# astaka-pe/Dual-DMP

Measured on NVIDIA B200. Metric: train iters/s (dual GCN fwd+bwd+loss+clip+Adam), higher is better.
Workload: dtype f32

## Files before the change

dual_dmp_b200/csrc/gemm_tc.cu:

```cuda
#include <cuda.h>
#include <cuda_fp16.h>
#include <stdlib.h>

#include <atomic>
#include <type_traits>

#include "common.cuh"

namespace ddmp {
namespace tc {

constexpr int kProducerWarps = 8;
constexpr int kProducerThreads = kProducerWarps * 32;
constexpr int BM = 128;
constexpr int BK = 32;
constexpr int UMMA_K = 8;

__device__ __forceinline__ uint32_t smem_u32(const void* p) { return (uint32_t)__cvta_generic_to_shared(p); }

__device__ __forceinline__ void mbar_init(uint64_t* bar, uint32_t count) {
    asm volatile("mbarrier.init.shared::cta.b64 [%0], %1;" ::"r"(smem_u32(bar)), "r"(count));
}
__device__ __forceinline__ void mbar_arrive(uint64_t* bar) {
    asm volatile("mbarrier.arrive.shared::cta.b64 _, [%0];" ::"r"(smem_u32(bar)) : "memory");
// ... 583 lines not shown
    auto load = [&](float4 (&buf)[NJ], uint32_t& vmask, int& k0) {
        k0 = lc_kb * BK16;
        vmask = 0;
#pragma unroll
        for (int j = 0; j < NJ; ++j) {
            if (rp[j]) {
                buf[j] = ldg4_pinned(rp[j] + k0);
                vmask |= 1u << j;
            } else {
                buf[j] = make_float4(0.f, 0.f, 0.f, 0.f);
            }
        }
        if (++lc_kb == num_kb) {
            lc_kb = 0;
            lc_tile += tile_step;
            if (lc_tile < g.num_tiles) set_rows(lc_tile);
        }
    };
    auto process = [&](float4 (&buf)[NJ], uint32_t vmask, int k0, uint32_t it) {
        const int s = it % STAGES;
        const uint32_t ph = (it / STAGES) & 1;
        const bool tr = g.trace && blockIdx.x == 0 && t == 0;
        long long c1 = 0, c2 = 0, c3 = 0;
        float4 sc = make_float4(s_a, s_a, s_a, s_a), sh = make_float4(0.f, 0.f, 0.f, 0.f);
        if (has_act) {
            sc = ldg4(g.scale + k0 + c8);
            sh = ldg4(g.shift + k0 + c8);
            sc.x *= s_a; sc.y *= s_a; sc.z *= s_a; sc.w *= s_a;
            sh.x *= s_a; sh.y *= s_a; sh.z *= s_a; sh.w *= s_a;
        }
        if (tr) c1 = clock64();
        wait_empty(empty_bar + s, ph ^ 1u);
        if (tr) c2 = clock64();
        const uint32_t st = smem_base + s * stage_bytes;
#pragma unroll
        for (int j = 0; j < NJ; ++j) {
            const uint32_t row = (t >> 4) + j * RPP;
            float4 a = buf[j];
            if (has_act) {
                if (vmask & (1u << j)) {
                    a.x = lrelu_max(fmaf(a.x, sc.x, sh.x), g.slope); a.y = lrelu_max(fmaf(a.y, sc.y, sh.y), g.slope);
                    a.z = lrelu_max(fmaf(a.z, sc.z, sh.z), g.slope); a.w = lrelu_max(fmaf(a.w, sc.w, sh.w), g.slope);
                }
            } else {
                a.x *= s_a; a.y *= s_a; a.z *= s_a; a.w *= s_a;
            }
            uint32_t h0, l0, h1, l1;
            split_f16x2(a.x, a.y, h0, l0);
            split_f16x2(a.z, a.w, h1, l1);
            const uint32_t off = sw128(row, c4 >> 1) + ((c4 & 1u) << 3);
            sts64(st + off, h0, h1);
            sts64(st + a_bytes + off, l0, l1);
        }
        long long cA = 0, cB = 0;
        if (tr) cA = clock64();
        fence_proxy_async();
        if (tr) cB = clock64();
        __syncwarp();
        if (tr) c3 = clock64();
        if (lane == 0) mbar_arrive(full_bar + s);
        if (tr) {
            g.trace[1] += (unsigned long long)(c2 - c1);
            g.trace[2] += (unsigned long long)(c3 - c2);
            g.trace[3] += 1ull;
            g.trace[14] += (unsigned long long)(cA - c2);
            g.trace[15] += (unsigned long long)(cB - cA);
        }
    };
    float4 buf0[NJ], buf1[NJ];
    uint32_t vm0 = 0, vm1 = 0;
    int k0 = 0, k1 = 0;
    if (total > 0) {
        set_rows(lc_tile);
        load(buf0, vm0, k0);
    }
    for (uint32_t it = 0; it < total; it += 2) {
        if (it + 1 < total) load(buf1, vm1, k1);
        process(buf0, vm0, k0, it);
        if (it + 1 >= total) break;
        if (it + 2 < total) load(buf0, vm0, k0);
        process(buf1, vm1, k1, it + 1);
    }
}
__device__ __forceinline__ void tmem_ld32_async(uint32_t taddr, uint32_t (&v)[32]) {
    asm volatile(
        "tcgen05.ld.sync.aligned.32x32b.x32.b32 "
        "{%0, %1, %2, %3, %4, %5, %6, %7, %8, %9, %10, %11, %12, %13, %14, %15, "
        "%16, %17, %18, %19, %20, %21, %22, %23, %24, %25, %26, %27, %28, %29, %30, %31}, [%32];\n"
        : "=r"(v[0]), "=r"(v[1]), "=r"(v[2]), "=r"(v[3]), "=r"(v[4]), "=r"(v[5]), "=r"(v[6]), "=r"(v[7]), "=r"(v[8]),
          "=r"(v[9]), "=r"(v[10]), "=r"(v[11]), "=r"(v[12]), "=r"(v[13]), "=r"(v[14]), "=r"(v[15]), "=r"(v[16]),
          "=r"(v[17]), "=r"(v[18]), "=r"(v[19]), "=r"(v[20]), "=r"(v[21]), "=r"(v[22]), "=r"(v[23]), "=r"(v[24]),
          "=r"(v[25]), "=r"(v[26]), "=r"(v[27]), "=r"(v[28]), "=r"(v[29]), "=r"(v[30]), "=r"(v[31])
        : "r"(taddr)
        : "memory");
}
__device__ __forceinline__ void tmem_wait_ld() { asm volatile("tcgen05.wait::ld.sync.aligned;" ::: "memory"); }

template <class Args>
__device__ __forceinline__ void epilogue_block32(const Args& g, uint32_t (&v)[32], float inv_sa, uint32_t stg, int lane,
                                                 int64_t mrow0, int ncol0) {
    const int cc = lane & 7;
    float4 w = ldg4(g.inv_sw + ncol0 + cc * 4);
    if (g.flags & 8) {
        const int64_t m = mrow0 + lane;
        if (m < g.M) {
#pragma unroll
            for (int i = 0; i < 8; ++i) {
                const float4 ws = ldg4(g.inv_sw + ncol0 + 4 * i);
                st4(g.C + m * g.N + ncol0 + 4 * i,
                    make_float4(__uint_as_float(v[4 * i]) * inv_sa * ws.x, __uint_as_float(v[4 * i + 1]) * inv_sa * ws.y,
                                __uint_as_float(v[4 * i + 2]) * inv_sa * ws.z, __uint_as_float(v[4 * i + 3]) * inv_sa * ws.w));
            }
        }
        return;
    }
#pragma unroll
    for (int i = 0; i < 8; ++i)
        sts128(stg + (uint32_t)lane * 128u + (uint32_t)((i ^ (lane & 7)) << 4),
               make_uint4(v[4 * i], v[4 * i + 1], v[4 * i + 2], v[4 * i + 3]));
    w.x *= inv_sa; w.y *= inv_sa; w.z *= inv_sa; w.w *= inv_sa;
    __syncwarp();
    uint4 o[8];
#pragma unroll
    for (int j = 0; j < 8; ++j) {
        const int r = j * 4 + (lane >> 3);
        asm volatile("ld.shared.v4.b32 {%0, %1, %2, %3}, [%4];"
                     : "=r"(o[j].x), "=r"(o[j].y), "=r"(o[j].z), "=r"(o[j].w)
                     : "r"(stg + (uint32_t)r * 128u + (uint32_t)((cc ^ (r & 7)) << 4)));
    }
#pragma unroll
    for (int j = 0; j < 8; ++j) {
        const int64_t m = mrow0 + j * 4 + (lane >> 3);
        if (m < g.M)
            st4(g.C + m * g.N + ncol0 + cc * 4,
                make_float4(__uint_as_float(o[j].x) * w.x, __uint_as_float(o[j].y) * w.y,
                            __uint_as_float(o[j].z) * w.z, __uint_as_float(o[j].w) * w.w));
    }
    __syncwarp();
}
template <int BN, class Args>
__device__ __forceinline__ void epilogue_tile(const Args& g, uint32_t taddr, float inv_sa, uint32_t stg, int lane,
                                              int64_t mrow0, int n0) {
    static_assert(BN % 64 == 0, "two 32-column blocks per iteration");
    uint32_t va[32], vb[32];
    tmem_ld32_async(taddr, va);
#pragma unroll 1
    for (int cb = 0; cb < BN; cb += 64) {
        const bool tr = g.trace && blockIdx.x == 0 && threadIdx.x == 12 * 32;
        long long q0 = 0;
        if (tr) q0 = clock64();
        tmem_wait_ld();
        if (tr) g.trace[13] += (unsigned long long)(clock64() - q0);
        tmem_ld32_async(taddr + (uint32_t)cb + 32u, vb);
        epilogue_block32(g, va, inv_sa, stg, lane, mrow0, n0 + cb);
        tmem_wait_ld();
        if (cb + 64 < BN) tmem_ld32_async(taddr + (uint32_t)cb + 64u, va);
        epilogue_block32(g, vb, inv_sa, stg, lane, mrow0, n0 + cb + 32);
    }
}

__device__ __forceinline__ void tma_store_2d(const CUtensorMap* map, uint32_t src_smem, int c0, int c1) {
    asm volatile("cp.async.bulk.tensor.2d.global.shared::cta.tile.bulk_group [%0, {%1, %2}], [%3];" ::"l"(map), "r"(c0),
                 "r"(c1), "r"(src_smem)
                 : "memory");
}
__device__ __forceinline__ void bulk_commit() { asm volatile("cp.async.bulk.commit_group;" ::: "memory"); }
// ... 11 lines not shown
#pragma unroll
    for (int i = 0; i < 8; ++i)
        sts128(stg + (uint32_t)lane * 128u + (uint32_t)((i ^ (lane & 7)) << 4),
               make_uint4(__float_as_uint(__uint_as_float(v[4 * i]) * (cs[i].x * inv_sa)),
                          __float_as_uint(__uint_as_float(v[4 * i + 1]) * (cs[i].y * inv_sa)),
                          __float_as_uint(__uint_as_float(v[4 * i + 2]) * (cs[i].z * inv_sa)),
                          __float_as_uint(__uint_as_float(v[4 * i + 3]) * (cs[i].w * inv_sa))));
    fence_proxy_async();
    __syncwarp();
    if (lane == 0) {
        tma_store_2d(cmap, stg, ncol0, mrow0);
        bulk_commit();
    }
}
template <int BN>
__device__ __forceinline__ void epilogue_tile_tma(const CUtensorMap* cmap, const float* __restrict__ inv_sw, uint32_t taddr,
                                                  float inv_sa, uint32_t stg, int lane, int64_t mrow0, int n0) {
    static_assert(BN % 64 == 0, "two 32-column blocks per iteration");
    uint32_t va[32], vb[32];
    float4 cs[8];
    tmem_ld32_async(taddr, va);
#pragma unroll 1
    for (int cb = 0; cb < BN; cb += 64) {
#pragma unroll
        for (int i = 0; i < 8; ++i) cs[i] = ldg4(inv_sw + n0 + cb + 4 * i);
        tmem_wait_ld();
        tmem_ld32_async(taddr + (uint32_t)cb + 32u, vb);
        store_block32_tma(cmap, va, cs, inv_sa, stg, lane, (int)mrow0, n0 + cb);
#pragma unroll
        for (int i = 0; i < 8; ++i) cs[i] = ldg4(inv_sw + n0 + cb + 32 + 4 * i);
        tmem_wait_ld();
        if (cb + 64 < BN) tmem_ld32_async(taddr + (uint32_t)cb + 64u, va);
        store_block32_tma(cmap, vb, cs, inv_sa, stg + 32u * 128u, lane, (int)mrow0, n0 + cb + 32);
    }
}

__global__ void tc_prep_b16_kernel(const float* __restrict__ W, int transposed, uint8_t* __restrict__ img,
                                   float* __restrict__ inv_sw, int N, int K, int BN) {
    const int n = (int)(((int64_t)blockIdx.x * blockDim.x + threadIdx.x) >> 5);
    const int lane = threadIdx.x & 31;
    if (n >= N) return;
    const int chunks = K / 8;
    auto load8 = [&](int c, float4& a, float4& b) {
        const int k = c * 8;
        if (!transposed) {
            a = ldg4(W + (int64_t)n * K + k);
            b = ldg4(W + (int64_t)n * K + k + 4);
        } else {
            a.x = __ldg(W + (int64_t)(k + 0) * N + n); a.y = __ldg(W + (int64_t)(k + 1) * N + n);
            a.z = __ldg(W + (int64_t)(k + 2) * N + n); a.w = __ldg(W + (int64_t)(k + 3) * N + n);
            b.x = __ldg(W + (int64_t)(k + 4) * N + n); b.y = __ldg(W + (int64_t)(k + 5) * N + n);
            b.z = __ldg(W + (int64_t)(k + 6) * N + n); b.w = __ldg(W + (int64_t)(k + 7) * N + n);
        }
    };
    uint32_t m = 0;
    for (int c = lane; c < chunks; c += 32) {
        float4 a, b;
        load8(c, a, b);
        const float mx = fmaxf(fmaxf(fmaxf(fabsf(a.x), fabsf(a.y)), fmaxf(fabsf(a.z), fabsf(a.w))),
                               fmaxf(fmaxf(fabsf(b.x), fabsf(b.y)), fmaxf(fabsf(b.z), fabsf(b.w))));
        const uint32_t bits = __float_as_uint(mx);
        m = bits > m ? bits : m;
    }
    m = __reduce_max_sync(0xffffffffu, m);
    float s, inv_s;
    scale_from_bits(m, s, inv_s);
    if (lane == 0) inv_sw[n] = inv_s;
    const int n_tile = n / BN, r = n % BN, num_kb = K / BK16;
    const int64_t half_bytes = (int64_t)BN * 128;
    for (int c = lane; c < chunks; c += 32) {
        float4 a, b;
        load8(c, a, b);
        a.x *= s; a.y *= s; a.z *= s; a.w *= s; b.x *= s; b.y *= s; b.z *= s; b.w *= s;
        uint4 hi, lo;
        split_f16x8(a, b, hi, lo);
        const int kb = c / 8, cc = c % 8;
        const int64_t base = ((int64_t)n_tile * num_kb + kb) * 2 * half_bytes;
        const uint32_t off = sw128((uint32_t)r, (uint32_t)cc);
        *reinterpret_cast<uint4*>(img + base + off) = hi;
        *reinterpret_cast<uint4*>(img + base + half_bytes + off) = lo;
    }
}

template <int BN, int STAGES>
__global__ void __launch_bounds__(kV2Threads, 1) tc_gemm_nt16_kernel(const __grid_constant__ CUtensorMap cmap,
                                                                     const Nt16Args g) {
    constexpr uint32_t A_BYTES = BM * 128;
    constexpr uint32_t B_BYTES = BN * 128;
    constexpr uint32_t STAGE_BYTES = 2 * A_BYTES + 2 * B_BYTES;
    constexpr uint32_t TMEM_COLS = 2 * BN;
    extern __shared__ __align__(1024) uint8_t smem_raw[];
    uint8_t* smem = reinterpret_cast<uint8_t*>((reinterpret_cast<uintptr_t>(smem_raw) + 1023) & ~(uintptr_t)1023);
    uint8_t* staging = smem + STAGES * STAGE_BYTES;
    uint64_t* full_bar = reinterpret_cast<uint64_t*>(staging + kStagingBytes);
    uint64_t* empty_bar = full_bar + STAGES;
    uint64_t* acc_full = empty_bar + STAGES;
    uint64_t* acc_empty = acc_full + 2;
    uint32_t* tmem_slot = reinterpret_cast<uint32_t*>(acc_empty + 2);
    uint32_t* amax_slot = tmem_slot + 1;

    const int warp = threadIdx.x >> 5, lane = threadIdx.x & 31;
    const int num_kb = g.K / BK16;
    if (threadIdx.x == 0) {
        for (int s = 0; s < STAGES; ++s) {
            mbar_init(full_bar + s, kProducerWarps + 1);
            mbar_init(empty_bar + s, 1);
        }
        for (int b = 0; b < 2; ++b) {
            mbar_init(acc_full + b, 1);
            mbar_init(acc_empty + b, 4);
        }
        *amax_slot = 0u;
        fence_barrier_init();
    }
    if (warp == 8) tmem_alloc(tmem_slot, TMEM_COLS);
    tc_fence_before();
    __syncthreads();
    tc_fence_after();
    block_amax_bits(g.amax, g.amax_len, amax_slot);
    __syncthreads();
    const uint32_t tmem_base = *tmem_slot;
    const uint32_t smem_base = smem_u32(smem);
    float s_a, inv_sa;
    scale_from_bits(*amax_slot, s_a, inv_sa);

    if (warp < kProducerWarps) {
        auto wait_empty = [](uint64_t* bar, uint32_t parity) { mbar_wait(bar, parity); };
        produce_loop<STAGES>(g, (int64_t)blockIdx.x, (int64_t)gridDim.x, (int64_t)BM, 0, num_kb, s_a,
                                        smem_base, STAGE_BYTES, A_BYTES, full_bar, empty_bar, wait_empty);
    } else if (warp == 8) {
        if (lane == 0) {
            constexpr uint32_t idesc = make_idesc16(BM, BN, false, false);
            uint32_t it = 0, tile_no = 0;
            for (int64_t tile = blockIdx.x; tile < g.num_tiles; tile += gridDim.x, ++tile_no) {
                const uint32_t buf = tile_no & 1u;
                mbar_wait(acc_empty + buf, ((tile_no >> 1) & 1u) ^ 1u);
                tc_fence_after();
                const uint32_t d_tmem = tmem_base + buf * BN;
                for (int kb = 0; kb < num_kb; ++kb, ++it) {
                    const int s = it % STAGES;
                    const uint32_t ph = (it / STAGES) & 1;
                    mbar_wait(full_bar + s, ph);
                    tc_fence_after();
                    const uint32_t sa = smem_base + s * STAGE_BYTES;
#pragma unroll
                    for (int ks = 0; ks < BK16 / UMMA_K16; ++ks) {
                        const uint32_t koff = ks * UMMA_K16 * 2;
                        const uint64_t a_hi = make_desc(sa + koff, 16, 1024);
                        const uint64_t a_lo = make_desc(sa + A_BYTES + koff, 16, 1024);
                        const uint64_t b_hi = make_desc(sa + 2 * A_BYTES + koff, 16, 1024);
                        const uint64_t b_lo = make_desc(sa + 2 * A_BYTES + B_BYTES + koff, 16, 1024);
                        umma_f16(d_tmem, a_lo, b_hi, idesc, (kb | ks) != 0);
                        umma_f16(d_tmem, a_hi, b_lo, idesc, 1);
                        umma_f16(d_tmem, a_hi, b_hi, idesc, 1);
                    }
                    umma_commit(empty_bar + s);
                }
                umma_commit(acc_full + buf);
            }
        }
        __syncwarp();
    } else if (warp == 9) {
        if (lane == 0) {
            uint32_t it = 0;
            for (int64_t tile = blockIdx.x; tile < g.num_tiles; tile += gridDim.x) {
                const int tn = (int)(tile % g.tiles_n);
                const uint8_t* src = g.Bimg + (int64_t)tn * num_kb * (2 * (int64_t)B_BYTES);
                for (int kb = 0; kb < num_kb; ++kb, ++it) {
                    const int s = it % STAGES;
                    const uint32_t ph = (it / STAGES) & 1;
                    mbar_wait(empty_bar + s, ph ^ 1u);
                    mbar_arrive_expect_tx(full_bar + s, 2 * B_BYTES);
                    bulk_g2s(smem_base + s * STAGE_BYTES + 2 * A_BYTES, src + (int64_t)kb * (2 * (int64_t)B_BYTES),
                             2 * B_BYTES, full_bar + s);
                }
            }
        }
        __syncwarp();
    } else if (warp >= 12) {
        const int q = warp & 3;
        const uint32_t stg = smem_u32(staging) + (uint32_t)q * kStageWarpBytes;
        const bool staged = (g.flags & 16) != 0;
        uint32_t tile_no = 0;
        for (int64_t tile = blockIdx.x; tile < g.num_tiles; tile += gridDim.x, ++tile_no) {
            const uint32_t buf = tile_no & 1u;
            const int64_t mrow0 = (tile / g.tiles_n) * BM + q * 32;
            const int n0 = (int)(tile % g.tiles_n) * BN;
            mbar_wait(acc_full + buf, (tile_no >> 1) & 1u);
            tc_fence_after();
            const uint32_t taddr = tmem_base + ((uint32_t)(q * 32) << 16) + buf * BN;
            if (staged) epilogue_tile<BN>(g, taddr, inv_sa, stg, lane, mrow0, n0);
            else epilogue_tile_tma<BN>(&cmap, g.inv_sw, taddr, inv_sa, stg, lane, mrow0, n0);
            tc_fence_before();
            __syncwarp();
            if (lane == 0) mbar_arrive(acc_empty + buf);
        }
        if (lane == 0) bulk_wait_all();
    }
    __syncthreads();
    if (warp == 8) {
        tc_fence_after();
        tmem_dealloc(tmem_base, TMEM_COLS);
    }
}

template <int BN, int STAGES>
static int launch_nt16(const Nt16Args& g, cudaStream_t st) {
    constexpr size_t smem = (size_t)STAGES * (2 * BM * 128 + 2 * BN * 128) + 1024 + 256 + kStagingBytes;
    static_assert(smem <= 232448, "shared memory of the fp16-split NT kernel");
    static PerDeviceOnce configured;
    if (configured.need()) {
        DDMP_CUDA(cudaFuncSetAttribute(tc_gemm_nt16_kernel<BN, STAGES>, cudaFuncAttributeMaxDynamicSharedMemorySize,
                                       (int)smem));
        configured.mark();
    }
    CUtensorMap cmap;
    int rc = make_tensor_map_2d(&cmap, g.C, g.M, g.N, 32, 32, true, "tc_gemm_nt16");
    if (rc != DDMP_OK) return rc;
    const int64_t grid = g.num_tiles < kNumSMs ? g.num_tiles : kNumSMs;
    tc_gemm_nt16_kernel<BN, STAGES><<<(unsigned)grid, kV2Threads, smem, st>>>(cmap, g);
    return check_launch("tc_gemm_nt16");
}

__device__ __forceinline__ void umma_f16_2cta(uint32_t tmem_d, uint64_t adesc, uint64_t bdesc, uint32_t idesc,
                                              uint32_t accumulate) {
    asm volatile(
        "{\n"
        ".reg .pred p;\n"
        "setp.ne.b32 p, %4, 0;\n"
        "tcgen05.mma.cta_group::2.kind::f16 [%0], %1, %2, %3, p;\n"
        "}\n" ::"r"(tmem_d),
        "l"(adesc), "l"(bdesc), "r"(idesc), "r"(accumulate)
        : "memory");
}

constexpr int kNt16x2Stages = 3;

__global__ void __cluster_dims__(2, 1, 1) __launch_bounds__(kV2Threads, 1)
tc_gemm_nt16x2_kernel(const __grid_constant__ CUtensorMap cmap, const Nt16Args g) {
    constexpr int STAGES = kNt16x2Stages;
    constexpr int BN = 256;
    constexpr uint32_t A_BYTES = BM * 128;
    constexpr uint32_t B_HALF = (BN / 2) * 128;
    constexpr uint32_t B_FULL = BN * 128;
    constexpr uint32_t STAGE_BYTES = 2 * A_BYTES + 2 * B_HALF;
    constexpr uint32_t TMEM_COLS = 2 * BN;
    extern __shared__ __align__(1024) uint8_t smem_raw[];
    uint8_t* smem = reinterpret_cast<uint8_t*>((reinterpret_cast<uintptr_t>(smem_raw) + 1023) & ~(uintptr_t)1023);
    uint8_t* staging = smem + STAGES * STAGE_BYTES;
    uint64_t* full_bar = reinterpret_cast<uint64_t*>(staging + kStagingBytes);
    uint64_t* empty_bar = full_bar + STAGES;
    uint64_t* peer_ready = empty_bar + STAGES;
    uint64_t* acc_full = peer_ready + STAGES;
    uint64_t* acc_empty = acc_full + 2;
    uint32_t* tmem_slot = reinterpret_cast<uint32_t*>(acc_empty + 2);
    uint32_t* amax_slot = tmem_slot + 1;

    const int warp = threadIdx.x >> 5, lane = threadIdx.x & 31;
    const uint32_t rank = cluster_ctarank();
    const int num_kb = g.K / BK16;
    const int64_t num_pairs = gridDim.x / 2, pair = blockIdx.x / 2;
    if (threadIdx.x == 0) {
        for (int s = 0; s < STAGES; ++s) {
            mbar_init(full_bar + s, kProducerWarps + 1);
            mbar_init(empty_bar + s, 1);
            mbar_init(peer_ready + s, 1);
        }
        for (int b = 0; b < 2; ++b) {
            mbar_init(acc_full + b, 1);
            mbar_init(acc_empty + b, 8);
        }
        *amax_slot = 0u;
        fence_barrier_init();
    }
    cluster_sync_all();
    if (warp == 8) tmem_alloc_2cta(tmem_slot, TMEM_COLS);
    tc_fence_before();
    __syncthreads();
    tc_fence_after();
    block_amax_bits(g.amax, g.amax_len, amax_slot);
    __syncthreads();
    const uint32_t tmem_base = *tmem_slot;
    const uint32_t smem_base = smem_u32(smem);
    float s_a, inv_sa;
    scale_from_bits(*amax_slot, s_a, inv_sa);

    if (warp < kProducerWarps) {
        auto wait_empty = [](uint64_t* bar, uint32_t parity) { mbar_wait_cluster(bar, parity); };
        produce_loop<STAGES>(g, pair, num_pairs, (int64_t)(2 * BM), (int64_t)rank * BM, num_kb, s_a,
                                        smem_base, STAGE_BYTES, A_BYTES, full_bar, empty_bar, wait_empty);
    } else if (warp == 8) {
        if (lane == 0) {
            uint32_t it = 0, tile_no = 0;
            if (rank == 0) {
                constexpr uint32_t idesc = make_idesc16(2 * BM, BN, false, false);
                for (int64_t tile = pair; tile < g.num_tiles; tile += num_pairs, ++tile_no) {
                    const uint32_t buf = tile_no & 1u;
                    long long a0 = 0;
                    if (g.trace && blockIdx.x == 0) a0 = clock64();
                    mbar_wait_cluster(acc_empty + buf, ((tile_no >> 1) & 1u) ^ 1u);
                    if (g.trace && blockIdx.x == 0) g.trace[7] += (unsigned long long)(clock64() - a0);
                    tc_fence_after();
                    const uint32_t d_tmem = tmem_base + buf * BN;
                    for (int kb = 0; kb < num_kb; ++kb, ++it) {
                        const int s = it % STAGES;
                        const uint32_t ph = (it / STAGES) & 1;
                        const bool tr = g.trace && blockIdx.x == 0;
                        long long c0 = 0, c1 = 0, c2 = 0;
                        if (tr) c0 = clock64();
                        mbar_wait(full_bar + s, ph);
                        if (tr) c1 = clock64();
                        mbar_wait_cluster(peer_ready + s, ph);
                        if (tr) {
                            c2 = clock64();
                            g.trace[4] += (unsigned long long)(c1 - c0);
                            g.trace[5] += (unsigned long long)(c2 - c1);
                            g.trace[6] += 1ull;
                        }
                        tc_fence_after();
                        const uint32_t sa = smem_base + s * STAGE_BYTES;
#pragma unroll
                        for (int ks = 0; ks < BK16 / UMMA_K16; ++ks) {
                            const uint32_t koff = ks * UMMA_K16 * 2;
                            const uint64_t a_hi = make_desc(sa + koff, 16, 1024);
                            const uint64_t a_lo = make_desc(sa + A_BYTES + koff, 16, 1024);
                            const uint64_t b_hi = make_desc(sa + 2 * A_BYTES + koff, 16, 1024);
                            const uint64_t b_lo = make_desc(sa + 2 * A_BYTES + B_HALF + koff, 16, 1024);
                            umma_f16_2cta(d_tmem, a_lo, b_hi, idesc, (kb | ks) != 0);
                            umma_f16_2cta(d_tmem, a_hi, b_lo, idesc, 1);
                            umma_f16_2cta(d_tmem, a_hi, b_hi, idesc, 1);
                        }
                        umma_commit_2cta(empty_bar + s);
                    }
                    umma_commit_2cta(acc_full + buf);
                }
            } else {
                for (int64_t tile = pair; tile < g.num_tiles; tile += num_pairs) {
                    for (int kb = 0; kb < num_kb; ++kb, ++it) {
                        const int s = it % STAGES;
                        const uint32_t ph = (it / STAGES) & 1;
                        mbar_wait(full_bar + s, ph);
                        mbar_arrive_remote(peer_ready + s, 0);
                    }
                }
            }
        }
        __syncwarp();
    } else if (warp == 9) {
        if (lane == 0) {
            uint32_t it = 0;
            for (int64_t tile = pair; tile < g.num_tiles; tile += num_pairs) {
                const int tn = (int)(tile % g.tiles_n);
                const uint8_t* src = g.Bimg + (int64_t)tn * num_kb * (2 * (int64_t)B_FULL) + (int64_t)rank * B_HALF;
                for (int kb = 0; kb < num_kb; ++kb, ++it) {
                    const int s = it % STAGES;
                    const uint32_t ph = (it / STAGES) & 1;
                    mbar_wait_cluster(empty_bar + s, ph ^ 1u);
                    mbar_arrive_expect_tx(full_bar + s, 2 * B_HALF);
                    const uint8_t* sk = src + (int64_t)kb * (2 * (int64_t)B_FULL);
                    const uint32_t dst = smem_base + s * STAGE_BYTES + 2 * A_BYTES;
                    bulk_g2s(dst, sk, B_HALF, full_bar + s);
                    bulk_g2s(dst + B_HALF, sk + B_FULL, B_HALF, full_bar + s);
                }
            }
        }
        __syncwarp();
    } else if (warp >= 12) {
        const int q = warp & 3;
        const uint32_t stg = smem_u32(staging) + (uint32_t)q * kStageWarpBytes;
        const bool staged = (g.flags & 16) != 0;
        uint32_t tile_no = 0;
        for (int64_t tile = pair; tile < g.num_tiles; tile += num_pairs, ++tile_no) {
            const uint32_t buf = tile_no & 1u;
            const int64_t mrow0 = (tile / g.tiles_n) * (2 * BM) + rank * BM + q * 32;
            const int n0 = (int)(tile % g.tiles_n) * BN;
            const bool tr = g.trace && blockIdx.x == 0 && warp == 12 && lane == 0;
            long long e0 = 0, e1 = 0;
            if (tr) e0 = clock64();
            mbar_wait_cluster(acc_full + buf, (tile_no >> 1) & 1u);
            if (tr) e1 = clock64();
            tc_fence_after();
            const uint32_t taddr = tmem_base + ((uint32_t)(q * 32) << 16) + buf * BN;
            if (staged) epilogue_tile<BN>(g, taddr, inv_sa, stg, lane, mrow0, n0);
            else epilogue_tile_tma<BN>(&cmap, g.inv_sw, taddr, inv_sa, stg, lane, mrow0, n0);
            tc_fence_before();
            __syncwarp();
            if (tr) {
                g.trace[8] += (unsigned long long)(e1 - e0);
                g.trace[9] += (unsigned long long)(clock64() - e1);
                g.trace[10] += 1ull;
            }
            if (lane == 0) {
                if (rank == 0) mbar_arrive(acc_empty + buf);
                else mbar_arrive_remote(acc_empty + buf, 0);
            }
        }
        if (lane == 0) bulk_wait_all();
    }
    tc_fence_before();
    cluster_sync_all();
    if (warp == 8) {
        tc_fence_after();
        tmem_dealloc_2cta(tmem_base, TMEM_COLS);
    }
}

static int launch_nt16x2(const Nt16Args& g0, cudaStream_t st) {
    constexpr size_t smem = (size_t)kNt16x2Stages * (2 * BM * 128 + 2 * 128 * 128) + 1024 + 256 + kStagingBytes;
    static_assert(smem <= 232448, "shared memory of the CTA-pair fp16-split NT kernel");
    static PerDeviceOnce configured;
    if (configured.need()) {
        DDMP_CUDA(cudaFuncSetAttribute(tc_gemm_nt16x2_kernel, cudaFuncAttributeMaxDynamicSharedMemorySize, (int)smem));
        configured.mark();
    }
    Nt16Args g = g0;
    g.num_tiles = ceil_div(g.M, 2 * BM) * g.tiles_n;
    CUtensorMap cmap;
    int rc = make_tensor_map_2d(&cmap, g.C, g.M, g.N, 32, 32, true, "tc_gemm_nt16x2");
    if (rc != DDMP_OK) return rc;
    const int64_t pairs = g.num_tiles < kNumSMs / 2 ? g.num_tiles : kNumSMs / 2;
    tc_gemm_nt16x2_kernel<<<(unsigned)(2 * pairs), kV2Threads, smem, st>>>(cmap, g);
    return check_launch("tc_gemm_nt16x2");
}

int f16_flags(int set) {
    static std::atomic<int> v{-1};
    int cur = v.load(std::memory_order_relaxed);
    if (cur < 0) {
        const char* e = getenv("DDMP_TC_F16_FLAGS");
        cur = e ? (atoi(e) & 0xffff) : 0;
        v.store(cur, std::memory_order_relaxed);
    }
    if (set >= 0) v.store(set & 0xffff, std::memory_order_relaxed);
    return cur;
}

static bool f16_split_enabled() {
    static const bool v = [] { const char* e = getenv("DDMP_TC_SPLIT"); return !(e && e[0] == 't'); }();
    return v;
}

static int run_nt16(const float* A, const int* a_map, const float* scale, const float* shift, float slope,
                    const float* W, int transposed, void* workspace, float* C, int64_t M, int N, int K,
                    const float* amax, int64_t amax_len, cudaStream_t st) {
    const int BN = (N % 256 == 0) ? 256 : ((N % 128 == 0) ? 128 : 64);
    uint8_t* img = reinterpret_cast<uint8_t*>(workspace);
    float* inv_sw = reinterpret_cast<float*>(img + (int64_t)N * K * 4);
    tc_prep_b16_kernel<<<(unsigned)ceil_div((int64_t)N * 32, 256), 256, 0, st>>>(W, transposed, img, inv_sw, N, K, BN);
    int rc = check_launch("tc_prep_b16");
    if (rc) return rc;
    Nt16Args g{};
    g.A = A; g.Bimg = img; g.inv_sw = inv_sw; g.C = C; g.a_map = a_map; g.scale = scale; g.shift = shift;
    g.slope = slope; g.amax = amax; g.amax_len = amax_len;
    g.flags = f16_flags(-1);
    if ((g.flags & 2) && K <= 256) g.flags |= 1;
    static const bool trace = [] { const char* e = getenv("DDMP_TC_TRACE"); return e && e[0] == '1'; }();
    static unsigned long long* trace_buf = nullptr;
    if (trace) {
        if (!trace_buf) cudaMalloc(&trace_buf, 16 * sizeof(unsigned long long));
        cudaMemsetAsync(trace_buf, 0, 16 * sizeof(unsigned long long), st);
        g.trace = trace_buf;
    }
    auto dump_trace = [&](int rc) {
        if (trace && rc == 0) {
            unsigned long long h[16];
            cudaStreamSynchronize(st);
            cudaMemcpy(h, trace_buf, sizeof(h), cudaMemcpyDeviceToHost);
            fprintf(stderr, "[ddmp trace] M=%lld N=%d K=%d | producer/stage: issue %llu wait_free %llu data+store %llu (n=%llu) | "
                    "mma/stage: wait_full %llu wait_peer %llu (n=%llu) wait_acc_total %llu | epilogue/tile: wait %llu drain %llu (n=%llu) "
                    "[to staging %llu, to global %llu, tmem wait(1 of 2) %llu] producer detail: transform+stores %llu fence %llu\n",
                    (long long)M, N, K, h[3] ? h[0] / h[3] : 0, h[3] ? h[1] / h[3] : 0, h[3] ? h[2] / h[3] : 0, h[3],
                    h[6] ? h[4] / h[6] : 0, h[6] ? h[5] / h[6] : 0, h[6], h[7], h[10] ? h[8] / h[10] : 0,
                    h[10] ? h[9] / h[10] : 0, h[10], h[10] ? h[11] / h[10] : 0, h[10] ? h[12] / h[10] : 0,
                    h[10] ? h[13] / h[10] : 0, h[3] ? h[14] / h[3] : 0, h[3] ? h[15] / h[3] : 0);
        }
        return rc;
    };
    g.M = M; g.N = N; g.K = K; g.tiles_n = N / BN;
    g.num_tiles = ceil_div(M, BM) * g.tiles_n;
    DDMP_REQUIRE(g.num_tiles < (1ll << 31), "tc gemm: too many tiles");
    static const bool one_cta = [] { const char* e = getenv("DDMP_TC_2CTA"); return e && e[0] == '0'; }();
    if (BN == 256 && !one_cta) return dump_trace(launch_nt16x2(g, st));
    if (BN == 256) return launch_nt16<256, 2>(g, st);
    if (BN == 128) return launch_nt16<128, 3>(g, st);
    return launch_nt16<64, 4>(g, st);
}

#ifndef DDMP_SEG_ROWS
#define DDMP_SEG_ROWS 2048
#endif
constexpr int kSegRows = DDMP_SEG_ROWS;

struct TnArgs {
    const float* A;
    const float* B;
    float* P;
    const float* scale;
    const float* shift;
    float slope;
    int64_t rows;
    int M, N;
    int tiles_m, tiles_n;
    int64_t num_items;
};

template <int BN, int STAGES, int PW>
__global__ void __launch_bounds__(PW * 32 + 32, 1) tc_gemm_tn_kernel(const TnArgs g) {
    constexpr int kPT = PW * 32;
    constexpr uint32_t A_BYTES = BM * 128;
    constexpr uint32_t B_BYTES = BN * 128;
    constexpr uint32_t STAGE_BYTES = 2 * A_BYTES + 2 * B_BYTES;
    constexpr uint32_t TMEM_COLS = BN < 32 ? 32 : BN;
    constexpr uint32_t LBO = (BK / 4) * 512;
    constexpr uint32_t SBO = 512;
    constexpr int A_CH = BM / 4, B_CH = BN / 4;
    extern __shared__ __align__(1024) uint8_t smem_raw[];
    uint8_t* smem = reinterpret_cast<uint8_t*>((reinterpret_cast<uintptr_t>(smem_raw) + 1023) & ~(uintptr_t)1023);
    uint64_t* full_bar = reinterpret_cast<uint64_t*>(smem + STAGES * STAGE_BYTES);
    uint64_t* empty_bar = full_bar + STAGES;
    uint64_t* accum_bar = empty_bar + STAGES;
    uint64_t* drained_bar = accum_bar + 1;
    uint32_t* tmem_slot = reinterpret_cast<uint32_t*>(drained_bar + 1);

    const int warp = threadIdx.x >> 5, lane = threadIdx.x & 31;
    if (threadIdx.x == 0) {
        for (int s = 0; s < STAGES; ++s) {
            mbar_init(full_bar + s, PW);
            mbar_init(empty_bar + s, 1);
        }
        mbar_init(accum_bar, 1);
        mbar_init(drained_bar, PW);
        fence_barrier_init();
    }
    if (warp == PW) tmem_alloc(tmem_slot, TMEM_COLS);
    tc_fence_before();
    __syncthreads();
    tc_fence_after();
    const uint32_t tmem_base = *tmem_slot;
    const uint32_t smem_base = smem_u32(smem);
    const int tiles = g.tiles_m * g.tiles_n;

    uint32_t it = 0;
    uint32_t item_no = 0;
    for (int64_t item = blockIdx.x; item < g.num_items; item += gridDim.x, ++item_no) {
        const int tile = (int)(item % tiles);
        const int64_t seg = item / tiles;
        const int m0 = (tile / g.tiles_n) * BM, n0 = (tile % g.tiles_n) * BN;
        const int64_t r0 = seg * kSegRows;
        const int64_t r1 = (r0 + kSegRows < g.rows) ? (r0 + kSegRows) : g.rows;
        const int num_kb = (int)((r1 - r0 + BK - 1) / BK);

        if (warp < PW) {
            const int t = threadIdx.x;
            const uint32_t a_cm = t % A_CH, a_r = t / A_CH;
            const uint32_t b_cm = t % B_CH, b_r = t / B_CH;
            constexpr int A_PASS = kPT / A_CH, B_PASS = kPT / B_CH;
            const bool a_ok = (m0 + (int)a_cm * 4) < g.M;
            const bool has_act = g.scale != nullptr;
            float4 sc = make_float4(1.f, 1.f, 1.f, 1.f), sh = make_float4(0.f, 0.f, 0.f, 0.f);
            if (has_act) { sc = ldg4(g.scale + n0 + b_cm * 4); sh = ldg4(g.shift + n0 + b_cm * 4); }
            const uint32_t a_off0 = (a_cm / 8) * LBO, b_off0 = (b_cm / 8) * LBO;
            float4 av[BK / A_PASS], bv[BK / B_PASS];
            auto issue = [&](int kb) {
                if (kb >= num_kb) return;
                const int64_t rb = r0 + (int64_t)kb * BK;
#pragma unroll
                for (int j = 0; j < BK / A_PASS; ++j) {
                    const int64_t r = rb + a_r + j * A_PASS;
// ... 698 lines not shown
```

Baseline: 16.71.

## Stage fp32 A tiles via TMA into raw smem before fp16-split transform

Adds a dedicated TMA warp that bulk-loads raw fp32 A tiles into a ring of shared-memory slots. The producer warps then read from shared memory, apply the scale/shift/leaky-ReLU and fp16 hi/lo split, and write the swizzled operand stage, instead of issuing global loads from registers. The aim is to take global-load latency off the producer critical path and to overlap the A fetch with the transform. It also raises TMEM accumulator buffering to 4 for the 1-CTA kernels, lowers the number of operand stages to make room for the raw slots, and prefers BN=128 over 256 for small K. The extra shared-memory use, fewer stages and the changed tile choice may reduce pipelining elsewhere.

```diff
diff --git a/dual_dmp_b200/csrc/gemm_tc.cu b/dual_dmp_b200/csrc/gemm_tc.cu
--- a/dual_dmp_b200/csrc/gemm_tc.cu
+++ b/dual_dmp_b200/csrc/gemm_tc.cu
@@ -689,6 +689,124 @@
         process(buf1, vm1, k1, it + 1);
     }
 }
+
+constexpr uint32_t kRawBoxBytes = BM * 128;
+constexpr uint32_t kRawSlotBytes = 2 * kRawBoxBytes;
+
+__device__ __forceinline__ void tma_load_2d(uint32_t dst_smem, const CUtensorMap* map, int c0, int c1, uint64_t* bar) {
+    asm volatile(
+        "cp.async.bulk.tensor.2d.shared::cluster.global.tile.mbarrier::complete_tx::bytes [%0], [%1, {%2, %3}], [%4];" ::"r"(
+            dst_smem),
+        "l"(map), "r"(c0), "r"(c1), "r"(smem_u32(bar))
+        : "memory");
+}
+__device__ __forceinline__ float4 lds128f(uint32_t saddr) {
+    float4 v;
+    asm volatile("ld.shared.v4.f32 {%0, %1, %2, %3}, [%4];" : "=f"(v.x), "=f"(v.y), "=f"(v.z), "=f"(v.w) : "r"(saddr)
+                 : "memory");
+    return v;
+}
+
+template <int RAW, class Args>
+__device__ __forceinline__ void tma_a_loop(const Args& g, const CUtensorMap* amap, int64_t first_tile, int64_t tile_step,
+                                           int64_t row_mul, int64_t row_add, int num_kb, uint32_t raw_base,
+                                           uint64_t* raw_full, uint64_t* raw_empty) {
+    const bool tr = g.trace && blockIdx.x == 0;
+    uint32_t it = 0;
+    for (int64_t tile = first_tile; tile < g.num_tiles; tile += tile_step) {
+        const int row0 = (int)((tile / g.tiles_n) * row_mul + row_add);
+        for (int kb = 0; kb < num_kb; ++kb, ++it) {
+            const int r = it % RAW;
+            const uint32_t rph = (it / RAW) & 1;
+            long long c0 = 0;
+            if (tr) c0 = clock64();
+            mbar_wait(raw_empty + r, rph ^ 1u);
+            if (tr) g.trace[12] += (unsigned long long)(clock64() - c0);
+            mbar_arrive_expect_tx(raw_full + r, kRawSlotBytes);
+            const uint32_t dst = raw_base + (uint32_t)r * kRawSlotBytes;
+            tma_load_2d(dst, amap, kb * BK16, row0, raw_full + r);
+            tma_load_2d(dst + kRawBoxBytes, amap, kb * BK16 + 32, row0, raw_full + r);
+        }
+    }
+}
+
+template <int STAGES, int RAW, class Args, class WaitEmpty>
+__device__ __forceinline__ void transform_loop(const Args& g, int64_t first_tile, int64_t tile_step, int num_kb, float s_a,
+                                               uint32_t smem_base, uint32_t raw_base, uint32_t stage_bytes,
+                                               uint32_t a_bytes, uint64_t* full_bar, uint64_t* empty_bar,
+                                               uint64_t* raw_full, uint64_t* raw_empty, WaitEmpty wait_empty) {
+    constexpr int NJ = kProdNJ, RPP = kProdRPP;
+    const int t = threadIdx.x, lane = threadIdx.x & 31;
+    const uint32_t c4 = t & 15;
+    const int c8 = (int)c4 * 4;
+    const bool has_act = g.scale != nullptr;
+    const bool tr = g.trace && blockIdx.x == 0 && t == 0;
+    const int64_t my_tiles = first_tile < g.num_tiles ? (g.num_tiles - first_tile + tile_step - 1) / tile_step : 0;
+    const uint32_t total = (uint32_t)(my_tiles * num_kb);
+    const uint32_t rd = raw_base + (c4 >> 3) * kRawBoxBytes;
+    int kb = 0;
+    for (uint32_t it = 0; it < total; ++it) {
+        const int s = it % STAGES, r = it % RAW;
+        const uint32_t ph = (it / STAGES) & 1, rph = (it / RAW) & 1;
+        const int k0 = kb * BK16;
+        if (++kb == num_kb) kb = 0;
+        long long c1 = 0, c2 = 0, c3 = 0, cA = 0, cB = 0, c4t = 0;
+        float4 sc = make_float4(s_a, s_a, s_a, s_a), sh = make_float4(0.f, 0.f, 0.f, 0.f);
+        if (has_act) {
+            sc = ldg4(g.scale + k0 + c8);
+            sh = ldg4(g.shift + k0 + c8);
+            sc.x *= s_a; sc.y *= s_a; sc.z *= s_a; sc.w *= s_a;
+            sh.x *= s_a; sh.y *= s_a; sh.z *= s_a; sh.w *= s_a;
+        }
+        if (tr) c1 = clock64();
+        mbar_wait(raw_full + r, rph);
+        if (tr) c2 = clock64();
+        const uint32_t raw = rd + (uint32_t)r * kRawSlotBytes;
+        float4 av[NJ];
+#pragma unroll
+        for (int j = 0; j < NJ; ++j) {
+            const uint32_t row = (t >> 4) + j * RPP;
+            av[j] = lds128f(raw + row * 128u + (((c4 & 7u) ^ (row & 7u)) << 4));
+        }
+        wait_empty(empty_bar + s, ph ^ 1u);
+        if (tr) c3 = clock64();
+        const uint32_t st = smem_base + s * stage_bytes;
+#pragma unroll
+        for (int j = 0; j < NJ; ++j) {
+            const uint32_t row = (t >> 4) + j * RPP;
+            float4 a = av[j];
+            if (has_act) {
+                a.x = lrelu_max(fmaf(a.x, sc.x, sh.x), g.slope); a.y = lrelu_max(fmaf(a.y, sc.y, sh.y), g.slope);
+                a.z = lrelu_max(fmaf(a.z, sc.z, sh.z), g.slope); a.w = lrelu_max(fmaf(a.w, sc.w, sh.w), g.slope);
+            } else {
+                a.x *= s_a; a.y *= s_a; a.z *= s_a; a.w *= s_a;
+            }
+            uint32_t h0, l0, h1, l1;
+            split_f16x2(a.x, a.y, h0, l0);
+            split_f16x2(a.z, a.w, h1, l1);
+            const uint32_t off = sw128(row, c4 >> 1) + ((c4 & 1u) << 3);
+            sts64(st + off, h0, h1);
+            sts64(st + a_bytes + off, l0, l1);
+        }
+        if (tr) cA = clock64();
+        fence_proxy_async();
+        if (tr) cB = clock64();
+        __syncwarp();
+        if (tr) c4t = clock64();
+        if (lane == 0) {
+            mbar_arrive(raw_empty + r);
+            mbar_arrive(full_bar + s);
+        }
+        if (tr) {
+            g.trace[11] += (unsigned long long)(c2 - c1);
+            g.trace[1] += (unsigned long long)(c3 - c2);
+            g.trace[2] += (unsigned long long)(c4t - c3);
+            g.trace[3] += 1ull;
+            g.trace[14] += (unsigned long long)(cA - c3);
+            g.trace[15] += (unsigned long long)(cB - cA);
+        }
+    }
+}
 __device__ __forceinline__ void tmem_ld32_async(uint32_t taddr, uint32_t (&v)[32]) {
     asm volatile(
         "tcgen05.ld.sync.aligned.32x32b.x32.b32 "
@@ -866,21 +984,26 @@
     }
 }
 
-template <int BN, int STAGES>
+template <int BN, int STAGES, int RAW, int ACC>
 __global__ void __launch_bounds__(kV2Threads, 1) tc_gemm_nt16_kernel(const __grid_constant__ CUtensorMap cmap,
+                                                                     const __grid_constant__ CUtensorMap amap,
                                                                      const Nt16Args g) {
     constexpr uint32_t A_BYTES = BM * 128;
     constexpr uint32_t B_BYTES = BN * 128;
     constexpr uint32_t STAGE_BYTES = 2 * A_BYTES + 2 * B_BYTES;
-    constexpr uint32_t TMEM_COLS = 2 * BN;
+    constexpr uint32_t TMEM_COLS = ACC * BN;
+    static_assert(TMEM_COLS <= 512 && (TMEM_COLS & (TMEM_COLS - 1)) == 0, "TMEM allocation: power of two <= 512");
     extern __shared__ __align__(1024) uint8_t smem_raw[];
     uint8_t* smem = reinterpret_cast<uint8_t*>((reinterpret_cast<uintptr_t>(smem_raw) + 1023) & ~(uintptr_t)1023);
-    uint8_t* staging = smem + STAGES * STAGE_BYTES;
+    uint8_t* raw = smem + STAGES * STAGE_BYTES;
+    uint8_t* staging = raw + RAW * kRawSlotBytes;
     uint64_t* full_bar = reinterpret_cast<uint64_t*>(staging + kStagingBytes);
     uint64_t* empty_bar = full_bar + STAGES;
     uint64_t* acc_full = empty_bar + STAGES;
-    uint64_t* acc_empty = acc_full + 2;
-    uint32_t* tmem_slot = reinterpret_cast<uint32_t*>(acc_empty + 2);
+    uint64_t* acc_empty = acc_full + ACC;
+    uint64_t* raw_full = acc_empty + ACC;
+    uint64_t* raw_empty = raw_full + RAW;
+    uint32_t* tmem_slot = reinterpret_cast<uint32_t*>(raw_empty + RAW);
     uint32_t* amax_slot = tmem_slot + 1;
 
     const int warp = threadIdx.x >> 5, lane = threadIdx.x & 31;
@@ -890,9 +1013,13 @@
             mbar_init(full_bar + s, kProducerWarps + 1);
             mbar_init(empty_bar + s, 1);
         }
-        for (int b = 0; b < 2; ++b) {
+        for (int b = 0; b < ACC; ++b) {
             mbar_init(acc_full + b, 1);
             mbar_init(acc_empty + b, 4);
+        }
+        for (int r = 0; r < RAW; ++r) {
+            mbar_init(raw_full + r, 1);
+            mbar_init(raw_empty + r, kProducerWarps);
         }
         *amax_slot = 0u;
         fence_barrier_init();
@@ -910,21 +1037,36 @@
 
     if (warp < kProducerWarps) {
         auto wait_empty = [](uint64_t* bar, uint32_t parity) { mbar_wait(bar, parity); };
-        produce_loop<STAGES>(g, (int64_t)blockIdx.x, (int64_t)gridDim.x, (int64_t)BM, 0, num_kb, s_a,
-                                        smem_base, STAGE_BYTES, A_BYTES, full_bar, empty_bar, wait_empty);
+        if constexpr (RAW > 0)
+            transform_loop<STAGES, RAW>(g, (int64_t)blockIdx.x, (int64_t)gridDim.x, num_kb, s_a, smem_base,
+                                        smem_u32(raw), STAGE_BYTES, A_BYTES, full_bar, empty_bar, raw_full, raw_empty,
+                                        wait_empty);
+        else
+            produce_loop<STAGES>(g, (int64_t)blockIdx.x, (int64_t)gridDim.x, (int64_t)BM, 0, num_kb, s_a,
+                                 smem_base, STAGE_BYTES, A_BYTES, full_bar, empty_bar, wait_empty);
     } else if (warp == 8) {
         if (lane == 0) {
             constexpr uint32_t idesc = make_idesc16(BM, BN, false, false);
+            const bool tr = g.trace && blockIdx.x == 0;
             uint32_t it = 0, tile_no = 0;
             for (int64_t tile = blockIdx.x; tile < g.num_tiles; tile += gridDim.x, ++tile_no) {
-                const uint32_t buf = tile_no & 1u;
-                mbar_wait(acc_empty + buf, ((tile_no >> 1) & 1u) ^ 1u);
+                const uint32_t buf = tile_no % ACC;
+                long long a0 = 0;
+                if (tr) a0 = clock64();
+                mbar_wait(acc_empty + buf, ((tile_no / ACC) & 1u) ^ 1u);
+                if (tr) g.trace[7] += (unsigned long long)(clock64() - a0);
                 tc_fence_after();
                 const uint32_t d_tmem = tmem_base + buf * BN;
                 for (int kb = 0; kb < num_kb; ++kb, ++it) {
                     const int s = it % STAGES;
                     const uint32_t ph = (it / STAGES) & 1;
+                    long long c0 = 0;
+                    if (tr) c0 = clock64();
                     mbar_wait(full_bar + s, ph);
+                    if (tr) {
+                        g.trace[4] += (unsigned long long)(clock64() - c0);
+                        g.trace[6] += 1ull;
+                    }
                     tc_fence_after();
                     const uint32_t sa = smem_base + s * STAGE_BYTES;
 #pragma unroll
@@ -961,22 +1103,41 @@
             }
         }
         __syncwarp();
+    } else if (warp == 10) {
+        if constexpr (RAW > 0) {
+            if (lane == 0)
+                tma_a_loop<RAW>(g, &amap, (int64_t)blockIdx.x, (int64_t)gridDim.x, (int64_t)BM, 0, num_kb, smem_u32(raw),
+                                raw_full, raw_empty);
+        }
+        __syncwarp();
     } else if (warp >= 12) {
         const int q = warp & 3;
         const uint32_t stg = smem_u32(staging) + (uint32_t)q * kStageWarpBytes;
         const bool staged = (g.flags & 16) != 0;
         uint32_t tile_no = 0;
         for (int64_t tile = blockIdx.x; tile < g.num_tiles; tile += gridDim.x, ++tile_no) {
-            const uint32_t buf = tile_no & 1u;
+            const uint32_t buf = tile_no % ACC;
             const int64_t mrow0 = (tile / g.tiles_n) * BM + q * 32;
             const int n0 = (int)(tile % g.tiles_n) * BN;
-            mbar_wait(acc_full + buf, (tile_no >> 1) & 1u);
+            const bool tr = g.trace && blockIdx.x == 0 && warp == 12 && lane == 0;
+            long long e0 = 0;
+            if (tr) e0 = clock64();
+            mbar_wait(acc_full + buf, (tile_no / ACC) & 1u);
+            if (tr) {
+                const long long e1 = clock64();
+                g.trace[8] += (unsigned long long)(e1 - e0);
+                g.trace[9] -= (unsigned long long)e1;
+            }
             tc_fence_after();
             const uint32_t taddr = tmem_base + ((uint32_t)(q * 32) << 16) + buf * BN;
             if (staged) epilogue_tile<BN>(g, taddr, inv_sa, stg, lane, mrow0, n0);
             else epilogue_tile_tma<BN>(&cmap, g.inv_sw, taddr, inv_sa, stg, lane, mrow0, n0);
             tc_fence_before();
             __syncwarp();
+            if (tr) {
+                g.trace[9] += (unsigned long long)clock64();
+                g.trace[10] += 1ull;
+            }
             if (lane == 0) mbar_arrive(acc_empty + buf);
         }
         if (lane == 0) bulk_wait_all();
@@ -988,21 +1149,31 @@
     }
 }
 
-template <int BN, int STAGES>
+constexpr size_t nt16_smem(int stages, uint32_t b_bytes, int raw) {
+    return (size_t)stages * (2 * BM * 128 + 2 * b_bytes) + (size_t)raw * kRawSlotBytes + kStagingBytes + 1024 + 256;
+}
+
+static int make_a_map(CUtensorMap* amap, const Nt16Args& g, const char* who) {
+    return make_tensor_map_2d(amap, g.A, g.M, g.K, BM, 32, true, who);
+}
+
+template <int BN, int STAGES, int RAW, int ACC>
 static int launch_nt16(const Nt16Args& g, cudaStream_t st) {
-    constexpr size_t smem = (size_t)STAGES * (2 * BM * 128 + 2 * BN * 128) + 1024 + 256 + kStagingBytes;
+    constexpr size_t smem = nt16_smem(STAGES, BN * 128, RAW);
     static_assert(smem <= 232448, "shared memory of the fp16-split NT kernel");
     static PerDeviceOnce configured;
     if (configured.need()) {
-        DDMP_CUDA(cudaFuncSetAttribute(tc_gemm_nt16_kernel<BN, STAGES>, cudaFuncAttributeMaxDynamicSharedMemorySize,
-                                       (int)smem));
+        DDMP_CUDA(cudaFuncSetAttribute(tc_gemm_nt16_kernel<BN, STAGES, RAW, ACC>,
+                                       cudaFuncAttributeMaxDynamicSharedMemorySize, (int)smem));
         configured.mark();
     }
     CUtensorMap cmap;
     int rc = make_tensor_map_2d(&cmap, g.C, g.M, g.N, 32, 32, true, "tc_gemm_nt16");
     if (rc != DDMP_OK) return rc;
+    CUtensorMap amap = cmap;
+    if (RAW > 0 && (rc = make_a_map(&amap, g, "tc_gemm_nt16 A")) != DDMP_OK) return rc;
     const int64_t grid = g.num_tiles < kNumSMs ? g.num_tiles : kNumSMs;
-    tc_gemm_nt16_kernel<BN, STAGES><<<(unsigned)grid, kV2Threads, smem, st>>>(cmap, g);
+    tc_gemm_nt16_kernel<BN, STAGES, RAW, ACC><<<(unsigned)grid, kV2Threads, smem, st>>>(cmap, amap, g);
     return check_launch("tc_gemm_nt16");
 }
 
@@ -1018,11 +1189,10 @@
         : "memory");
 }
 
-constexpr int kNt16x2Stages = 3;
-
+template <int STAGES, int RAW>
 __global__ void __cluster_dims__(2, 1, 1) __launch_bounds__(kV2Threads, 1)
-tc_gemm_nt16x2_kernel(const __grid_constant__ CUtensorMap cmap, const Nt16Args g) {
-    constexpr int STAGES = kNt16x2Stages;
+tc_gemm_nt16x2_kernel(const __grid_constant__ CUtensorMap cmap, const __grid_constant__ CUtensorMap amap,
+                      const Nt16Args g) {
     constexpr int BN = 256;
     constexpr uint32_t A_BYTES = BM * 128;
     constexpr uint32_t B_HALF = (BN / 2) * 128;
@@ -1031,13 +1201,16 @@
     constexpr uint32_t TMEM_COLS = 2 * BN;
     extern __shared__ __align__(1024) uint8_t smem_raw[];
     uint8_t* smem = reinterpret_cast<uint8_t*>((reinterpret_cast<uintptr_t>(smem_raw) + 1023) & ~(uintptr_t)1023);
-    uint8_t* staging = smem + STAGES * STAGE_BYTES;
+    uint8_t* raw = smem + STAGES * STAGE_BYTES;
+    uint8_t* staging = raw + RAW * kRawSlotBytes;
     uint64_t* full_bar = reinterpret_cast<uint64_t*>(staging + kStagingBytes);
     uint64_t* empty_bar = full_bar + STAGES;
     uint64_t* peer_ready = empty_bar + STAGES;
     uint64_t* acc_full = peer_ready + STAGES;
     uint64_t* acc_empty = acc_full + 2;
-    uint32_t* tmem_slot = reinterpret_cast<uint32_t*>(acc_empty + 2);
+    uint64_t* raw_full = acc_empty + 2;
+    uint64_t* raw_empty = raw_full + RAW;
+    uint32_t* tmem_slot = reinterpret_cast<uint32_t*>(raw_empty + RAW);
     uint32_t* amax_slot = tmem_slot + 1;
 
     const int warp = threadIdx.x >> 5, lane = threadIdx.x & 31;
@@ -1053,6 +1226,10 @@
         for (int b = 0; b < 2; ++b) {
             mbar_init(acc_full + b, 1);
             mbar_init(acc_empty + b, 8);
+        }
+        for (int r = 0; r < RAW; ++r) {
+            mbar_init(raw_full + r, 1);
+            mbar_init(raw_empty + r, kProducerWarps);
         }
         *amax_slot = 0u;
         fence_barrier_init();
@@ -1071,8 +1248,12 @@
 
     if (warp < kProducerWarps) {
         auto wait_empty = [](uint64_t* bar, uint32_t parity) { mbar_wait_cluster(bar, parity); };
-        produce_loop<STAGES>(g, pair, num_pairs, (int64_t)(2 * BM), (int64_t)rank * BM, num_kb, s_a,
-                                        smem_base, STAGE_BYTES, A_BYTES, full_bar, empty_bar, wait_empty);
+        if constexpr (RAW > 0)
+            transform_loop<STAGES, RAW>(g, pair, num_pairs, num_kb, s_a, smem_base, smem_u32(raw), STAGE_BYTES, A_BYTES,
+                                        full_bar, empty_bar, raw_full, raw_empty, wait_empty);
+        else
+            produce_loop<STAGES>(g, pair, num_pairs, (int64_t)(2 * BM), (int64_t)rank * BM, num_kb, s_a,
+                                 smem_base, STAGE_BYTES, A_BYTES, full_bar, empty_bar, wait_empty);
     } else if (warp == 8) {
         if (lane == 0) {
             uint32_t it = 0, tile_no = 0;
@@ -1149,6 +1330,13 @@
             }
         }
         __syncwarp();
+    } else if (warp == 10) {
+        if constexpr (RAW > 0) {
+            if (lane == 0)
+                tma_a_loop<RAW>(g, &amap, pair, num_pairs, (int64_t)(2 * BM), (int64_t)rank * BM, num_kb, smem_u32(raw),
+                                raw_full, raw_empty);
+        }
+        __syncwarp();
     } else if (warp >= 12) {
         const int q = warp & 3;
         const uint32_t stg = smem_u32(staging) + (uint32_t)q * kStageWarpBytes;
@@ -1159,10 +1347,14 @@
             const int64_t mrow0 = (tile / g.tiles_n) * (2 * BM) + rank * BM + q * 32;
             const int n0 = (int)(tile % g.tiles_n) * BN;
             const bool tr = g.trace && blockIdx.x == 0 && warp == 12 && lane == 0;
-            long long e0 = 0, e1 = 0;
+            long long e0 = 0;
             if (tr) e0 = clock64();
             mbar_wait_cluster(acc_full + buf, (tile_no >> 1) & 1u);
-            if (tr) e1 = clock64();
+            if (tr) {
+                const long long e1 = clock64();
+                g.trace[8] += (unsigned long long)(e1 - e0);
+                g.trace[9] -= (unsigned long long)e1;
+            }
             tc_fence_after();
             const uint32_t taddr = tmem_base + ((uint32_t)(q * 32) << 16) + buf * BN;
             if (staged) epilogue_tile<BN>(g, taddr, inv_sa, stg, lane, mrow0, n0);
@@ -1170,8 +1362,7 @@
             tc_fence_before();
             __syncwarp();
             if (tr) {
-                g.trace[8] += (unsigned long long)(e1 - e0);
-                g.trace[9] += (unsigned long long)(clock64() - e1);
+                g.trace[9] += (unsigned long long)clock64();
                 g.trace[10] += 1ull;
             }
             if (lane == 0) {
@@ -1189,12 +1380,14 @@
     }
 }
 
+template <int STAGES, int RAW>
 static int launch_nt16x2(const Nt16Args& g0, cudaStream_t st) {
-    constexpr size_t smem = (size_t)kNt16x2Stages * (2 * BM * 128 + 2 * 128 * 128) + 1024 + 256 + kStagingBytes;
+    constexpr size_t smem = nt16_smem(STAGES, 128 * 128, RAW);
     static_assert(smem <= 232448, "shared memory of the CTA-pair fp16-split NT kernel");
     static PerDeviceOnce configured;
     if (configured.need()) {
-        DDMP_CUDA(cudaFuncSetAttribute(tc_gemm_nt16x2_kernel, cudaFuncAttributeMaxDynamicSharedMemorySize, (int)smem));
+        DDMP_CUDA(cudaFuncSetAttribute(tc_gemm_nt16x2_kernel<STAGES, RAW>, cudaFuncAttributeMaxDynamicSharedMemorySize,
+                                       (int)smem));
         configured.mark();
     }
     Nt16Args g = g0;
@@ -1202,8 +1395,10 @@
     CUtensorMap cmap;
     int rc = make_tensor_map_2d(&cmap, g.C, g.M, g.N, 32, 32, true, "tc_gemm_nt16x2");
     if (rc != DDMP_OK) return rc;
+    CUtensorMap amap = cmap;
+    if (RAW > 0 && (rc = make_a_map(&amap, g, "tc_gemm_nt16x2 A")) != DDMP_OK) return rc;
     const int64_t pairs = g.num_tiles < kNumSMs / 2 ? g.num_tiles : kNumSMs / 2;
-    tc_gemm_nt16x2_kernel<<<(unsigned)(2 * pairs), kV2Threads, smem, st>>>(cmap, g);
+    tc_gemm_nt16x2_kernel<STAGES, RAW><<<(unsigned)(2 * pairs), kV2Threads, smem, st>>>(cmap, amap, g);
     return check_launch("tc_gemm_nt16x2");
 }
 
@@ -1227,7 +1422,10 @@
 static int run_nt16(const float* A, const int* a_map, const float* scale, const float* shift, float slope,
                     const float* W, int transposed, void* workspace, float* C, int64_t M, int N, int K,
                     const float* amax, int64_t amax_len, cudaStream_t st) {
-    const int BN = (N % 256 == 0) ? 256 : ((N % 128 == 0) ? 128 : 64);
+    int flags = f16_flags(-1);
+    if ((flags & 2) && K <= 256) flags |= 1;
+    const bool tma_a = (K <= 256 || scale != nullptr) && a_map == nullptr && !(flags & 32) && M < (1ll << 31) - 2 * BM;
+    const int BN = (N % 256 == 0 && !(tma_a && K <= 128)) ? 256 : ((N % 128 == 0) ? 128 : 64);
     uint8_t* img = reinterpret_cast<uint8_t*>(workspace);
     float* inv_sw = reinterpret_cast<float*>(img + (int64_t)N * K * 4);
     tc_prep_b16_kernel<<<(unsigned)ceil_div((int64_t)N * 32, 256), 256, 0, st>>>(W, transposed, img, inv_sw, N, K, BN);
@@ -1236,8 +1434,7 @@
     Nt16Args g{};
     g.A = A; g.Bimg = img; g.inv_sw = inv_sw; g.C = C; g.a_map = a_map; g.scale = scale; g.shift = shift;
     g.slope = slope; g.amax = amax; g.amax_len = amax_len;
-    g.flags = f16_flags(-1);
-    if ((g.flags & 2) && K <= 256) g.flags |= 1;
+    g.flags = flags;
     static const bool trace = [] { const char* e = getenv("DDMP_TC_TRACE"); return e && e[0] == '1'; }();
     static unsigned long long* trace_buf = nullptr;
     if (trace) {
@@ -1250,13 +1447,14 @@
             unsigned long long h[16];
             cudaStreamSynchronize(st);
             cudaMemcpy(h, trace_buf, sizeof(h), cudaMemcpyDeviceToHost);
-            fprintf(stderr, "[ddmp trace] M=%lld N=%d K=%d | producer/stage: issue %llu wait_free %llu data+store %llu (n=%llu) | "
-                    "mma/stage: wait_full %llu wait_peer %llu (n=%llu) wait_acc_total %llu | epilogue/tile: wait %llu drain %llu (n=%llu) "
-                    "[to staging %llu, to global %llu, tmem wait(1 of 2) %llu] producer detail: transform+stores %llu fence %llu\n",
-                    (long long)M, N, K, h[3] ? h[0] / h[3] : 0, h[3] ? h[1] / h[3] : 0, h[3] ? h[2] / h[3] : 0, h[3],
-                    h[6] ? h[4] / h[6] : 0, h[6] ? h[5] / h[6] : 0, h[6], h[7], h[10] ? h[8] / h[10] : 0,
-                    h[10] ? h[9] / h[10] : 0, h[10], h[10] ? h[11] / h[10] : 0, h[10] ? h[12] / h[10] : 0,
-                    h[10] ? h[13] / h[10] : 0, h[3] ? h[14] / h[3] : 0, h[3] ? h[15] / h[3] : 0);
+            auto per = [](unsigned long long x, unsigned long long n) { return n ? x / n : 0ull; };
+            fprintf(stderr, "[ddmp trace] M=%lld N=%d K=%d A=%s | producer/kb: wait_raw %llu wait_free %llu data+store %llu "
+                    "(n=%llu) [transform+stores %llu fence %llu] | tma_a/kb: wait_slot %llu | mma/kb: wait_full %llu "
+                    "wait_peer %llu (n=%llu) | mma/tile: wait_acc %llu | epilogue/tile: wait %llu drain %llu (n=%llu) "
+                    "[staged tmem wait %llu]\n",
+                    (long long)M, N, K, tma_a ? "tma" : "registers", per(h[11], h[3]), per(h[1], h[3]), per(h[2], h[3]),
+                    h[3], per(h[14], h[3]), per(h[15], h[3]), per(h[12], h[3]), per(h[4], h[6]), per(h[5], h[6]), h[6],
+                    per(h[7], h[10]), per(h[8], h[10]), per(h[9], h[10]), h[10], per(h[13], h[10]));
         }
         return rc;
     };
@@ -1264,10 +1462,15 @@
     g.num_tiles = ceil_div(M, BM) * g.tiles_n;
     DDMP_REQUIRE(g.num_tiles < (1ll << 31), "tc gemm: too many tiles");
     static const bool one_cta = [] { const char* e = getenv("DDMP_TC_2CTA"); return e && e[0] == '0'; }();
-    if (BN == 256 && !one_cta) return dump_trace(launch_nt16x2(g, st));
-    if (BN == 256) return launch_nt16<256, 2>(g, st);
-    if (BN == 128) return launch_nt16<128, 3>(g, st);
-    return launch_nt16<64, 4>(g, st);
+    if (BN == 256 && one_cta) return dump_trace(launch_nt16<256, 2, 0, 2>(g, st));
+    if (tma_a) {
+        if (BN == 256) return dump_trace(launch_nt16x2<2, 2>(g, st));
+        if (BN == 128) return dump_trace(launch_nt16<128, 2, 2, 4>(g, st));
+        return dump_trace(launch_nt16<64, 2, 3, 4>(g, st));
+    }
+    if (BN == 256) return dump_trace(launch_nt16x2<3, 0>(g, st));
+    if (BN == 128) return dump_trace(launch_nt16<128, 3, 0, 2>(g, st));
+    return dump_trace(launch_nt16<64, 4, 0, 2>(g, st));
 }
 
 #ifndef DDMP_SEG_ROWS
```

Result: faster. 17.28, median of 6 (+3.4%).
